# MicahZoltu/lodestar

Hardware: AMD Instinct MI355X
Metric: verified signature sets/sec (mainnet attestation mix) (higher is better)
Workload: dtype u32 (381-bit Montgomery; device products on 14x28-bit limbs); 1 GPU; c3: gossip attestation flood, 6 slot(s) per batch, 7 batches in flight per GPU; slots_per_batch=6, sets_per_gpu=116736, jobs_per_gpu=104448, pubkeys_per_gpu=1683456, parallelism=dp1 (sets sharded), exchange=False, inflight=7, world_size_seen=1, pubkeys=indices into the GPU-resident table, signing_roots_per_gpu=6918

## Files before the change

lodestar_amd/csrc/lb_engine.hip:

```cpp
#include <hip/hip_runtime.h>
#include <hip/hip_ext.h>
#include <stdio.h>
#include <stdlib.h>
#include <string.h>
#include <sys/random.h>

#include <algorithm>
#include <chrono>
#include <cstdio>
#include <cstdlib>
#include <atomic>
#include <mutex>
#include <string>
#include <vector>

#include "lb_kernels.h"
#include "lb_engine_impl.h"
#include "lb_kdecl.h"
#include "lb_search_plan.h"

#define LB_ABI_VERSION 1

namespace {
const char* const kStageNames[kStages] = {"decode_sigs", "dedup",   "hash_map", "hash_finish", "pk_chunks",
// ... 635 lines not shown
                         e->bacc.as<uint32_t>(), bcap, e->bsum.as<uint32_t>(), nb);
    hipLaunchKernelGGL(k_msm_window_g8, dim3(n_inst * W), dim3(256), 0, st, e->bsum.as<uint32_t>(), nb,
                       e->wsum.as<uint32_t>(), n_inst * W);
    if (W == LB_MSM_W)
      hipLaunchKernelGGL(k_msm_horner_g8<LB_MSM_W>, dim3((n_inst + 7) / 8), dim3(64), 0, st, e->wsum.as<uint32_t>(),
                         n_inst, out, n_out, out0);
    else
      hipLaunchKernelGGL(k_msm_horner_g8<LB_SMSM_W>, dim3((n_inst + 7) / 8), dim3(64), 0, st, e->wsum.as<uint32_t>(),
                         n_inst, out, n_out, out0);
    return hipGetLastError();
  }
  hipLaunchKernelGGL(k_msm_buckets, dim3(nblk(nb)), dim3(LB_TPB), 0, st, e->bch.as<uint32_t>(), e->bacc.as<uint32_t>(),
                     bcap, e->bsum.as<uint32_t>(), nb);
  if (W == LB_MSM_W)
    hipLaunchKernelGGL(k_msm_reduce<LB_MSM_W>, dim3(n_inst), dim3(64 * LB_MSM_W), 0, st, e->bsum.as<uint32_t>(), nb, out,
                       n_out, out0);
  else
    hipLaunchKernelGGL(k_msm_reduce<LB_SMSM_W>, dim3(n_inst), dim3(64 * LB_SMSM_W), 0, st, e->bsum.as<uint32_t>(), nb,
                       out, n_out, out0);
  return hipGetLastError();
}

static hipError_t per_root_chain(lb_engine* e, uint32_t n, uint32_t nuh, uint32_t mu) {
  hipStream_t s1 = e->stream;
  const uint32_t* nu = e->n_u.as<uint32_t>();
  const bool row = e->alone && e->row_fe;
  const bool row_roots = row && nuh <= e->row_max;
  {
    stage_scope sc(e, ST_GSUM, s1);
    const uint32_t nch = nuh + n / e->gchunk;
    if (e->alone)
      hipLaunchKernelGGL(k_gsum_wave, dim3(nblk(nch)), dim3(LB_TPB), 0, s1, n, nu, e->gch.as<uint32_t>(),
                         e->chunk_beg.as<uint32_t>(), e->chunk_end.as<uint32_t>(), e->chunk_root.as<uint32_t>(),
                         e->members.as<uint32_t>(), e->set_live.as<uint32_t>(), e->rpk.as<uint32_t>(), e->gacc.as<uint32_t>());
    else
      hipLaunchKernelGGL(k_gsum_chunks, dim3(nblk(nch)), dim3(LB_TPB), 0, s1, n, nu,
                         e->gch.as<uint32_t>(), e->chunk_beg.as<uint32_t>(), e->chunk_end.as<uint32_t>(),
                         e->members.as<uint32_t>(), e->set_live.as<uint32_t>(), e->rpk.as<uint32_t>(), e->gacc.as<uint32_t>());
    hipLaunchKernelGGL(k_gsum_final, dim3(nblk_inv(nuh)), dim3(LB_INV_TPB), 0, s1, n, nu, e->gch.as<uint32_t>(),
                       e->gacc.as<uint32_t>(), e->gp_aff.as<uint32_t>(), e->gp_inf.as<uint32_t>(),
                       e->alone ? 1u : 0u);
  }
  {
    stage_scope sc(e, ST_MILLER, s1);
    const bool shared = e->miller_form == 1 ||
                        (e->miller_form == 0 && !device_alone(e));
    if (row_roots) {
      hipLaunchKernelGGL(k_miller_row, dim3(nuh), dim3(LBR_NT), 0, s1, n, mu, nu, e->gp_aff.as<uint32_t>(),
                         e->gp_inf.as<uint32_t>(), e->h_aff.as<uint32_t>(), e->treeP.as<uint32_t>());
    } else if (nuh <= e->miller_wave_max) {
      hipLaunchKernelGGL(k_miller_wave, dim3(nuh), dim3(64), 0, s1, n, mu, nu, e->gp_aff.as<uint32_t>(),
                         e->gp_inf.as<uint32_t>(), e->h_aff.as<uint32_t>(), e->treeP.as<uint32_t>());
    } else if (shared) {
      hipError_t r = e->park.ensure((size_t)2 * 72 * 4 * n);
      if (r != hipSuccess) return r;
      if (nuh <= e->miller_lds3_max)
        hipLaunchKernelGGL(k_miller_lane<3>, dim3(nblk(nuh)), dim3(LB_TPB), 0, s1, n, mu, nu, e->gp_aff.as<uint32_t>(),
                           e->gp_inf.as<uint32_t>(), e->h_aff.as<uint32_t>(), e->treeP.as<uint32_t>(),
                           e->park.as<uint32_t>());
      else
        hipLaunchKernelGGL(k_miller_lane<2>, dim3(nblk(nuh)), dim3(LB_TPB), 0, s1, n, mu, nu, e->gp_aff.as<uint32_t>(),
                           e->gp_inf.as<uint32_t>(), e->h_aff.as<uint32_t>(), e->treeP.as<uint32_t>(),
                           e->park.as<uint32_t>());
    } else {
      hipLaunchKernelGGL(k_miller_g8, dim3((nuh + LBG_ROOTS - 1) / LBG_ROOTS), dim3(64 * LBG_WAVES), 0, s1, n, mu, nu,
                         e->gp_aff.as<uint32_t>(), e->gp_inf.as<uint32_t>(), e->h_aff.as<uint32_t>(),
                         e->treeP.as<uint32_t>());
    }
  }
  {
    stage_scope sc(e, ST_TREE_P, s1);
    for (uint32_t lo = mu / 2; lo >= 1; lo /= 2) {
      if (row && lo <= e->row_max)
        hipLaunchKernelGGL(k_tree_up_row, dim3(lo), dim3(LBR_NT), 0, s1, mu, lo, nu, e->treeP.as<uint32_t>());
      else
        hipLaunchKernelGGL(k_tree_up_U, dim3(lo), dim3(64), 0, s1, mu, lo, nu, e->treeP.as<uint32_t>());
    }
  }
  return hipGetLastError();
}

static int32_t run_pipeline(lb_engine* e, lb_batch* b, const uint64_t* scalars, uint32_t& mj, uint32_t& mu,
                            bool unblinded) {
  const uint32_t n = b->n_sets, nj = b->n_jobs;
  e->partial_serial = 0;
  e->alone = device_alone(e);
  e->gchunk = e->alone ? LB_GROUP_CHUNK_WAVE : LB_GROUP_CHUNK;
  const bool row = e->alone && e->row_fe;
  const bool row_small = row && n <= e->row_max;
  const bool one_unblinded = n == 1 && !scalars && unblinded;
  int st = fill_scalars(e, n, scalars, unblinded);
  if (st != LB_OK) return st;
  mj = 1;
  while (mj < nj) mj <<= 1;
  mu = 1;
  while (mu < n) mu <<= 1;
  const uint32_t mt = mj > mu ? mj : mu;
  const uint32_t ns = n ? n : 1;
  uint32_t cap = 64;
  while (cap < 2 * ns) cap <<= 1;
  LB_HIP(e->scalars.ensure((size_t)ns * 8));
  LB_HIP(e->sig_aff.ensure((size_t)ns * sizeof(g2a)));
  LB_HIP(e->sig_inf.ensure((size_t)ns * 4));
  LB_HIP(e->sig_status.ensure((size_t)ns * 4));
  LB_HIP(e->q.ensure((size_t)ns * 2 * sizeof(g2j)));
  LB_HIP(e->h_aff.ensure((size_t)ns * sizeof(g2a)));
  LB_HIP(e->rpk.ensure((size_t)ns * sizeof(g1j)));
// ... 872 lines not shown
```

lodestar_amd/csrc/lb_field.h:

```cpp
#pragma once
#include "lb_common.h"
#include "lb_consts.h"

struct fp {
  uint32_t v[12];
};
struct fp2 {
  fp c0, c1;
};
struct fp6 {
  fp2 c0, c1, c2;
};
struct fp12 {
  fp6 c0, c1;
};

LB_HD fp fp_load(const uint32_t* c) {
  fp r;
  LB_UNROLL for (int i = 0; i < 12; i++) r.v[i] = c[i];
  return r;
}
LB_HD fp2 fp2_load(const uint32_t* c) {
  fp2 r;
  r.c0 = fp_load(c);
// ... 451 lines not shown
  const uint32_t P28[14] = {LB_P28_0, LB_P28_1, LB_P28_2, LB_P28_3, LB_P28_4,  LB_P28_5,  LB_P28_6,
                            LB_P28_7, LB_P28_8, LB_P28_9, LB_P28_10, LB_P28_11, LB_P28_12, LB_P28_13};
  typedef unsigned __int128 u128;
  const u128 lim = (u128)~0ull;
  fp28_chk_in(a), fp28_chk_in(b);
  if (c) fp28_chk_in(*c), fp28_chk_in(*d);
  u128 col[29];
  for (int k = 0; k < 29; k++) col[k] = 0;
  for (int i = 0; i < 14; i++) {
    for (int j = 0; j < 14; j++) {
      col[i + j] += (u128)a.ub[i] * b.ub[j] + (u128)0x0fffffffu * P28[j];
      if (c) col[i + j] += (u128)c->ub[i] * d->ub[j];
    }
    LB_CHK_ASSERT(col[i] <= lim);
    col[i + 1] += col[i] >> 28;
  }
  for (int k = 14; k < 28; k++) {
    LB_CHK_ASSERT(col[k] <= lim);
    col[k + 1] += col[k] >> 28;
  }
  const double s = a.vb * b.vb + (c ? c->vb * d->vb : 0.0);
  const double vb = (1.0 + s / 2520.0) * (1.0 + 1e-9);
  LB_CHK_ASSERT(vb < 2520.0);
  fp28_chk_set(r, vb);
}
#endif

struct fp2_28 {
  fp28 c0, c1;
};
LB_HD fp28 fp28_add(const fp28& a, const fp28& b) {
  fp28 r;
  LB_UNROLL for (int k = 0; k < 14; k++) {
    r.l[k] = a.l[k] + b.l[k];
    LB_CHK(r.ub[k] = a.ub[k] + b.ub[k]; LB_CHK_ASSERT(r.ub[k] <= 0xffffffffull);)
  }
  LB_CHK(r.vb = a.vb + b.vb;)
  return r;
}
template <int N>
LB_HD fp28 fp28_muls(const fp28& a) {
  fp28 r;
  LB_UNROLL for (int k = 0; k < 14; k++) {
    r.l[k] = N == 3 ? (a.l[k] << 1) + a.l[k] : a.l[k] << (N == 2 ? 1 : N == 4 ? 2 : 3);
    LB_CHK(r.ub[k] = N * a.ub[k]; LB_CHK_ASSERT(r.ub[k] <= 0xffffffffull);)
  }
  LB_CHK(r.vb = N * a.vb;)
  return r;
}
template <uint32_t C, int S>
LB_HD fp28 fp28_kminus(const fp28& b) {
  constexpr uint32_t K[14] = LB_K28(C, S);
  fp28 r;
  LB_UNROLL for (int k = 0; k < 14; k++) {
    r.l[k] = K[k] - b.l[k];
    LB_CHK(LB_CHK_ASSERT(b.ub[k] <= K[k]); r.ub[k] = K[k];)
  }
  LB_CHK(r.vb = C;)
  return r;
}
template <uint32_t C, int S>
LB_HD fp28 fp28_sub(const fp28& a, const fp28& b) {
  constexpr uint32_t K[14] = LB_K28(C, S);
  fp28 r;
  LB_UNROLL for (int k = 0; k < 14; k++) {
    r.l[k] = a.l[k] + K[k] - b.l[k];
    LB_CHK(LB_CHK_ASSERT(b.ub[k] <= K[k]); r.ub[k] = a.ub[k] + K[k]; LB_CHK_ASSERT(r.ub[k] <= 0xffffffffull);)
  }
  LB_CHK(r.vb = a.vb + C;)
  return r;
}
LB_HD fp28 fp28_norm(const fp28& a) {
  fp28 r;
  uint32_t c = 0;
  LB_CHK(uint64_t cb = 0;)
  LB_UNROLL for (int k = 0; k < 13; k++) {
    const uint32_t t = a.l[k] + c;
    LB_CHK(LB_CHK_ASSERT(a.ub[k] + cb <= 0xffffffffull); cb = (a.ub[k] + cb) >> 28;)
    r.l[k] = t & 0x0fffffffu;
    c = t >> 28;
  }
  r.l[13] = a.l[13] + c;
  LB_CHK(const uint64_t top = a.ub[13] + cb; fp28_chk_set(r, a.vb); if (top < r.ub[13]) r.ub[13] = top;)
  return r;
}
LB_HD fp28 fp28_mulx(const fp28& a, const fp28& b) {
#if defined(__HIP_DEVICE_COMPILE__)
  __builtin_amdgcn_sched_barrier(0);
#endif
  fp28 r = fp28_mul_raw(a, b);
#if defined(__HIP_DEVICE_COMPILE__)
  __builtin_amdgcn_sched_barrier(0);
#endif
  LB_CHK(fp28_chk_mac(a, b, nullptr, nullptr, r);)
  return r;
}
LB_HD fp28 fp28_mac2(const fp28& a, const fp28& b, const fp28& c, const fp28& d) {
  const uint32_t P28[14] = {LB_P28_0, LB_P28_1, LB_P28_2, LB_P28_3, LB_P28_4,  LB_P28_5,  LB_P28_6,
                            LB_P28_7, LB_P28_8, LB_P28_9, LB_P28_10, LB_P28_11, LB_P28_12, LB_P28_13};
#if defined(__HIP_DEVICE_COMPILE__)
  __builtin_amdgcn_sched_barrier(0);
#endif
  uint64_t acc[28];
  LB_UNROLL for (int k = 0; k < 28; k++) acc[k] = 0;
  LB_UNROLL for (int i = 0; i < 14; i++) {
    LB_UNROLL for (int j = 0; j < 14; j++) {
      LB_COL_CHK(acc[i + j], a.l[i], b.l[j]);
      acc[i + j] += (uint64_t)a.l[i] * b.l[j];
    }
    LB_UNROLL for (int j = 0; j < 14; j++) {
      LB_COL_CHK(acc[i + j], c.l[i], d.l[j]);
      acc[i + j] += (uint64_t)c.l[i] * d.l[j];
    }
    const uint32_t m = ((uint32_t)acc[i] * LB_PINV28) & 0x0fffffffu;
    LB_UNROLL for (int j = 0; j < 14; j++) {
      LB_COL_CHK(acc[i + j], m, P28[j]);
      acc[i + j] += (uint64_t)m * P28[j];
// ... 59 lines not shown
  }
  return fp_reduce_once(o, 0u);
}
LB_HD bool fp28_is_zero(const fp28& a) {
  const uint32_t P28[14] = {LB_P28_0, LB_P28_1, LB_P28_2, LB_P28_3, LB_P28_4,  LB_P28_5,  LB_P28_6,
                            LB_P28_7, LB_P28_8, LB_P28_9, LB_P28_10, LB_P28_11, LB_P28_12, LB_P28_13};
  LB_CHK(fp28_chk_in(a); LB_CHK_ASSERT(a.vb < 2520.0);)
  uint64_t acc[28];
  LB_UNROLL for (int k = 0; k < 28; k++) acc[k] = k < 14 ? a.l[k] : 0;
  LB_UNROLL for (int i = 0; i < 14; i++) {
    const uint32_t m = ((uint32_t)acc[i] * LB_PINV28) & 0x0fffffffu;
    LB_UNROLL for (int j = 0; j < 14; j++) acc[i + j] += (uint64_t)m * P28[j];
    acc[i + 1] += acc[i] >> 28;
  }
  uint32_t z = 0, e = 0;
  LB_UNROLL for (int k = 0; k < 14; k++) {
    const uint32_t t = k < 13 ? ((uint32_t)acc[14 + k] & 0x0fffffffu) : (uint32_t)acc[27];
    if (k < 13) acc[15 + k] += acc[14 + k] >> 28;
    z |= t;
    e |= t ^ P28[k];
  }
  return z == 0 || e == 0;
}

LB_HD fp2_28 fp2_28_add(const fp2_28& a, const fp2_28& b) { return fp2_28{fp28_add(a.c0, b.c0), fp28_add(a.c1, b.c1)}; }
template <int N>
LB_HD fp2_28 fp2_28_muls(const fp2_28& a) {
  return fp2_28{fp28_muls<N>(a.c0), fp28_muls<N>(a.c1)};
}
template <uint32_t C, int S>
LB_HD fp2_28 fp2_28_sub(const fp2_28& a, const fp2_28& b) {
  return fp2_28{fp28_sub<C, S>(a.c0, b.c0), fp28_sub<C, S>(a.c1, b.c1)};
}
LB_HD fp2_28 fp2_28_norm(const fp2_28& a) { return fp2_28{fp28_norm(a.c0), fp28_norm(a.c1)}; }
template <uint32_t C, int S>
LB_HD fp2_28 fp2_28_mul(const fp2_28& a, const fp2_28& b) {
  const fp28 nb1 = fp28_kminus<C, S>(b.c1);
  fp2_28 r;
  r.c0 = fp28_mac2(a.c0, b.c0, a.c1, nb1);
  r.c1 = fp28_mac2(a.c0, b.c1, a.c1, b.c0);
  return r;
}
template <uint32_t C, int S>
LB_HD fp2_28 fp2_28_sqr(const fp2_28& a) {
  fp2_28 r;
  r.c0 = fp28_mulx(fp28_add(a.c0, a.c1), fp28_sub<C, S>(a.c0, a.c1));
  r.c1 = fp28_mulx(fp28_muls<2>(a.c0), a.c1);
  return r;
}
LB_HD bool fp2_28_is_zero(const fp2_28& a) { return fp28_is_zero(a.c0) & fp28_is_zero(a.c1); }
LB_HD fp2_28 fp2_28_from_fp2(const fp2& a) { return fp2_28{fp28_from_fp(a.c0), fp28_from_fp(a.c1)}; }
LB_HD fp2_28 fp2_28_from_fp2_shift(const fp2& a) { return fp2_28{fp28_from_fp_shift(a.c0), fp28_from_fp_shift(a.c1)}; }
LB_HD fp2 fp2_28_to_fp2(const fp2_28& a) { return fp2{fp28_to_fp(a.c0), fp28_to_fp(a.c1)}; }

template <bool kInlMul = false>
LB_HD fp fp_pow_const_i(fp a, const uint32_t* e, int top_bit) {
  if constexpr (kInlMul) return fp_pow_const_28(a, e, top_bit);
  fp tab[8];
  tab[0] = a;
  const fp a2 = fp_sqr(a);
  LB_UNROLL for (int k = 1; k < 8; k++) tab[k] = fp_mul(tab[k - 1], a2);
  auto bit = [&](int i) -> uint32_t { return (e[i >> 5] >> (i & 31)) & 1u; };
  fp r = fp_zero();
  bool first = true;
  int i = top_bit;
  while (i >= 0) {
    if (!bit(i)) {
      r = fp_sqr(r);
      i--;
      continue;
    }
    int j = i - 3 > 0 ? i - 3 : 0;
    while (!bit(j)) j++;
    uint32_t val = 0;
    for (int k = i; k >= j; k--) val = (val << 1) | bit(k);
    if (first) {
      r = lb_tab8(tab, val >> 1);
      first = false;
    } else {
      for (int k = i; k >= j; k--) r = fp_sqr(r);
      r = fp_mul(r, lb_tab8(tab, val >> 1));
    }
    i = j - 1;
  }
  return r;
}

LB_HD bool lb_is_one_plain(const uint32_t* x) {
  uint32_t t = x[0] ^ 1u;
  LB_UNROLL for (int i = 1; i < 12; i++) t |= x[i];
  return t == 0;
}
LB_HD int lb_ctz32(uint32_t x) {
#if defined(__HIP_DEVICE_COMPILE__)
  return __builtin_ctz(x);
#else
  return __builtin_ctz(x);
#endif
}
LB_HD void lb_shr(uint32_t* u, int k) {
  LB_UNROLL for (int j = 0; j < 11; j++) u[j] = (u[j] >> k) | (u[j + 1] << (32 - k));
  u[11] >>= k;
}
LB_HD bool lb_geq(const uint32_t* a, const uint32_t* b) {
  uint32_t br = 0;
  LB_UNROLL for (int j = 0; j < 12; j++) (void)LB_SUBC(a[j], b[j], br, &br);
// ... 585 lines not shown
```

lodestar_amd/csrc/lb_kernels.h:

```cpp
#pragma once
#include "lb_serial.h"
#include "lb_h2c.h"
#include "lb_pairing.h"

#define LB_TPB 64
#ifndef LB_MINW
#define LB_MINW 1
#endif
#ifndef LB_MINW_DEC
#define LB_MINW_DEC 2
#endif
#ifndef LB_MINW_SUB
#define LB_MINW_SUB LB_MINW_DEC
#endif
#ifndef LB_MINW_MSM
#define LB_MINW_MSM 1
#endif
#ifndef LB_MINW_GSUM
#define LB_MINW_GSUM 1
#endif
typedef fpi lb_g1f;
typedef fp2i lb_g2f;
typedef jac<lb_g2f> g2jm;
#ifndef LB_MINW_G1
// ... 972 lines not shown
    ok = g2_aff_in_subgroup_i(P);
  } else {
    const rfp2 Z2 = f_sqr(Z);
    const rfp2 sx = f_mul(fl_conj(px), fl_in(fp2_load(LB_PSI_CX), t2));
    const rfp2 sy = f_mul(fl_conj(py), fl_in(fp2_load(LB_PSI_CY), t2));
    ok = fp2_eq(fl_out(f_mul(sx, Z2)), fl_out(X)) && fp2_eq(fl_out(f_mul(f_mul(sy, Z2), Z)), fl_out(f_neg(Y)));
  }
  if (!ok && threadIdx.x == 0) sig_status[i] = LB_POINT_NOT_IN_GROUP;
}
#endif
#if LB_KG(13)
__global__ void __launch_bounds__(64) k_sig_blind_w4(uint32_t n, const uint32_t* __restrict__ sig_aff,
                                                    const uint64_t* __restrict__ scalars,
                                                    const uint32_t* __restrict__ sig_inf, uint32_t* __restrict__ terms) {
  const uint32_t i = blockIdx.x;
  if (i >= n) return;
  const uint64_t w = scalars[i];
  g2j r = jac_infinity<fp2>();
  if (!sig_inf[i] && w != 0) {
    const g2a S = soa_ld<g2a>(sig_aff, n, i);
    const rfp2* t2p = nullptr;
    const rfp* t1p = nullptr;
    const rfp2 x1 = fl_in(S.x, t2p), y1 = fl_in(S.y, t2p);
    const rfp c2x = fl_in(fp_load(LB_PSI2_CX), t1p), c2y = fl_in(fp_load(LB_PSI2_CY), t1p);
    const rfp c4x = fl_in(fp_load(LB_PSI4_CX), t1p), c4y = fl_in(fp_load(LB_PSI4_CY), t1p);
    const rfp2 x2 = fl_mulb(x1, c2x), y2 = f_neg(fl_mulb(y1, c2y));
    const rfp2 x3 = fl_mulb(x1, c4x), y3 = f_neg(fl_mulb(y1, c4y));
    const uint32_t k0 = (uint32_t)w, k1 = (uint32_t)(w >> 32);
    auto digit = [&](int b) { return ((k0 >> b) & 1u) | (((k1 >> b) & 1u) << 1); };
    int b = 31;
    while (b > 0 && digit(b) == 0) b--;
    const uint32_t d0 = digit(b);
    rfp2 X = d0 == 1u ? x1 : (d0 == 2u ? x2 : x3), Y = d0 == 1u ? y1 : (d0 == 2u ? y2 : y3), Z;
    f_set_one(Z);
#pragma clang loop unroll(disable)
    for (b--; b >= 0; b--) {
      w4_g2_dbl(X, Y, Z);
      const uint32_t d = digit(b);
      if (d != 0u) w4_g2_madd(X, Y, Z, d == 1u ? x1 : (d == 2u ? x2 : x3), d == 1u ? y1 : (d == 2u ? y2 : y3));
    }
    r = g2j{fl_out(X), fl_out(Y), fl_out(Z)};
  }
  if (threadIdx.x == 0) soa_st(terms, n, i, r);
}
#endif

typedef __attribute__((address_space(3))) uint32_t lds_w;
template <int NL>
struct lane_lds {
  lds_w* L;
  uint32_t* g;
  uint32_t n, u;
  int lane;
  __device__ __forceinline__ void put(int k, const fp6& v) const {
    const uint32_t* w = reinterpret_cast<const uint32_t*>(&v);
    if (k < NL)
      LB_UNROLL for (int i = 0; i < 72; i++) L[(k * 72 + i) * 64 + lane] = w[i];
    else
      LB_UNROLL for (int i = 0; i < 72; i++) g[((size_t)(k - 2) * 72 + i) * n + u] = w[i];
    __asm__ volatile("" ::: "memory");
  }
  __device__ __forceinline__ fp6 get(int k) const {
    __asm__ volatile("" ::: "memory");
    fp6 v;
    uint32_t* w = reinterpret_cast<uint32_t*>(&v);
    if (k < NL)
      LB_UNROLL for (int i = 0; i < 72; i++) w[i] = L[(k * 72 + i) * 64 + lane];
    else
      LB_UNROLL for (int i = 0; i < 72; i++) w[i] = g[((size_t)(k - 2) * 72 + i) * n + u];
    return v;
  }
};
template <class S_t>
__device__ __forceinline__ void lane_f_sqr(const S_t& S) {
  fp6 s1, s2;
  {
    const fp6 a0 = S.get(0), a1 = S.get(1);
    S.put(2, fp6_mul_inl(a0, a1));
    s1 = fp6_add(a0, a1);
    s2 = fp6_add(a0, fp6_mul_v(a1));
  }
  const fp6 c0 = fp6_mul_inl(s1, s2);
  const fp6 t = S.get(2);
  S.put(0, fp6_sub(fp6_sub(c0, t), fp6_mul_v(t)));
  S.put(1, fp6_add(t, t));
}
template <class S_t>
__device__ __forceinline__ void lane_f_line(const S_t& S, const fp2& l0, const fp2& l2, const fp2& l3) {
  fp6 s;
  {
    const fp6 a1 = S.get(1);
    S.put(2, fp6_mul_1(a1, l3));
    const fp6 a0 = S.get(0);
    s = fp6_add(a0, a1);
    S.put(0, fp6_mul_01(a0, l0, l2));
  }
  const fp6 c1 = fp6_mul_01(s, l0, fp2_add(l2, l3));
  const fp6 t0 = S.get(0), t1 = S.get(2);
  S.put(1, fp6_sub(fp6_sub(c1, t0), t1));
  S.put(0, fp6_add(t0, fp6_mul_v(t1)));
}
#if LB_KG(4)
template <int NL>
__global__ void __launch_bounds__(LB_TPB, 1) k_miller_lane(uint32_t n, uint32_t m,
                                                           const uint32_t* __restrict__ n_u,
                                                           const uint32_t* __restrict__ gp_aff,
                                                           const uint32_t* __restrict__ gp_inf,
                                                           const uint32_t* __restrict__ h_aff,
                                                           uint32_t* __restrict__ treeP, uint32_t* __restrict__ tpark) {
  static_assert(LB_TPB == 64, "one wave per block: 64 lanes of LDS slots");
  __shared__ uint32_t lds[NL * 72 * 64];
  const uint32_t u = lb_tid();
  if (u >= *n_u) return;
  const lane_lds<NL> S{(lds_w*)lds, tpark, n, u, (int)threadIdx.x};
  S.put(0, fp6_one());
  S.put(1, fp6_zero());
  if (!gp_inf[u]) {
    auto park_t = [&](const g2j& T) { S.put(3, *reinterpret_cast<const fp6*>(&T)); };
    auto unpark_t = [&]() {
      const fp6 v = S.get(3);
      return *reinterpret_cast<const g2j*>(&v);
    };
    {
      const g2a Q = soa_ld<g2a>(h_aff, n, u);
      park_t(g2j{Q.x, Q.y, fp2_one()});
    }
    bool first = true;
#pragma clang loop unroll(disable)
    for (int i = 62; i >= 0; i--) {
      if (!first) lane_f_sqr(S);
      first = false;
      fp2 l0, l2, l3;
      {
        g2j T = unpark_t();
        const g1a P = soa_ld<g1a>(gp_aff, n, u);
        miller_dbl(T, l0, l2, l3, P.x, P.y);
        park_t(T);
      }
      lane_f_line(S, l0, l2, l3);
      if ((LB_X_ABS >> i) & 1ull) {
        {
          g2j T = unpark_t();
          const g1a P = soa_ld<g1a>(gp_aff, n, u);
          miller_add(T, soa_ld<g2a>(h_aff, n, u), l0, l2, l3, P.x, P.y);
          park_t(T);
        }
        lane_f_line(S, l0, l2, l3);
      }
    }
    S.put(1, fp6_neg(S.get(1)));
  }
  LB_UNROLL for (int h = 0; h < 2; h++) {
    const fp6 v = S.get(h);
    const uint32_t* w = reinterpret_cast<const uint32_t*>(&v);
    LB_UNROLL for (int i = 0; i < 72; i++) treeP[(size_t)(72 * h + i) * (2 * m) + m + u] = w[i];
  }
}
#endif

#if LB_KG(5)
__global__ void __launch_bounds__(64) k_miller_wave(uint32_t n, uint32_t m, const uint32_t* __restrict__ n_u,
                                                    const uint32_t* __restrict__ gp_aff,
                                                    const uint32_t* __restrict__ gp_inf,
                                                    const uint32_t* __restrict__ h_aff, uint32_t* __restrict__ treeP) {
  LBW_SHARED_MILLER(S);
  const uint32_t u = blockIdx.x;
  if (u >= *n_u) return;
  const int lane = threadIdx.x;
  w_init_consts(S, LBW_MILLER_COUNT, LBW_MILLER_FIRST);
  const bool inf = gp_inf[u] != 0;
  if (inf) {
    w_set_one(S, LBW_A(0));
  } else {
    if (lane < 6) {
      const uint32_t* base = lane < 2 ? gp_aff + (size_t)12 * lane * n : h_aff + (size_t)12 * (lane - 2) * n;
      fp v;
      LB_UNROLL for (int w = 0; w < 12; w++) v.v[w] = base[(size_t)w * n + u];
      w_st(S, LBW_PT + lane, v);
    }
    w_sync();
    w_miller(S, LBW_A(0));
  }
  w_store_soa12(S, LBW_A(0), treeP, 2 * m, m + u);
}
#endif

#define LB_GROUP_CHUNK 32
#ifndef LB_GROUP_CHUNK_WAVE
#define LB_GROUP_CHUNK_WAVE 4
#endif
#ifndef LB_MSM_CHUNK
#define LB_MSM_CHUNK 16
#endif
__device__ __forceinline__ bool msg_eq(const uint8_t* __restrict__ msgs, uint32_t a, uint32_t b) {
  const uint4* x = reinterpret_cast<const uint4*>(msgs + (size_t)32 * a);
  const uint4* y = reinterpret_cast<const uint4*>(msgs + (size_t)32 * b);
  const uint4 x0 = x[0], x1 = x[1], y0 = y[0], y1 = y[1];
  return ((x0.x ^ y0.x) | (x0.y ^ y0.y) | (x0.z ^ y0.z) | (x0.w ^ y0.w) | (x1.x ^ y1.x) | (x1.y ^ y1.y) |
          (x1.z ^ y1.z) | (x1.w ^ y1.w)) == 0u;
}
__device__ __forceinline__ uint32_t msg_hash(const uint8_t* __restrict__ msgs, uint32_t i, uint64_t key) {
  const uint4* x = reinterpret_cast<const uint4*>(msgs + (size_t)32 * i);
  const uint4 a = x[0], b = x[1];
  const uint32_t w[8] = {a.x, a.y, a.z, a.w, b.x, b.y, b.z, b.w};
  uint64_t h = key;
  LB_UNROLL for (int k = 0; k < 8; k++) {
    h = (h ^ w[k]) * 0x9E3779B97F4A7C15ull;
    h ^= h >> 29;
// ... 1452 lines not shown
```

lodestar_amd/csrc/lb_pairing.h:

```cpp
#pragma once
#include "lb_curve.h"

template <bool kInl = false>
LB_HD void miller_dbl(g2j& T, fp2& l0, fp2& l2, fp2& l3, const fp& xP, const fp& yP) {
  fp2 X = T.x, Y = T.y, Z = T.z;
  fp2 A = lean2_mul<kInl>(X, Y);
  fp2 B = lean2_sqr<kInl>(Y);
  fp2 C = lean2_sqr<kInl>(Z);
  fp2 E = fp2_mul3(fp2_dbl(fp2_dbl(fp2_mul_xi(C))));
  fp2 F = fp2_mul3(E);
  fp2 H = fp2_sub(lean2_sqr<kInl>(fp2_add(Y, Z)), fp2_add(B, C));
  fp2 XX3 = fp2_mul3(lean2_sqr<kInl>(X));
  l0 = fp2_sub(B, E);
  l2 = fp2_neg(fp2{lean_mul<kInl>(XX3.c0, xP), lean_mul<kInl>(XX3.c1, xP)});
  l3 = fp2{lean_mul<kInl>(H.c0, yP), lean_mul<kInl>(H.c1, yP)};
  T.x = fp2_dbl(lean2_mul<kInl>(A, fp2_sub(B, F)));
  T.y = fp2_sub(lean2_sqr<kInl>(fp2_add(B, F)), fp2_mul3(fp2_dbl(fp2_dbl(lean2_sqr<kInl>(E)))));
  T.z = fp2_dbl(fp2_dbl(lean2_mul<kInl>(B, H)));
}

template <bool kInl = false>
LB_HD void miller_add(g2j& T, const g2a& Q, fp2& l0, fp2& l2, fp2& l3, const fp& xP, const fp& yP) {
  fp2 theta = fp2_sub(T.y, lean2_mul<kInl>(Q.y, T.z));
  fp2 lam = fp2_sub(T.x, lean2_mul<kInl>(Q.x, T.z));
// ... 9 lines not shown
  T.x = lean2_mul<kInl>(lam, H);
  T.y = fp2_sub(lean2_mul<kInl>(theta, fp2_sub(G, H)), lean2_mul<kInl>(E, T.y));
  T.z = lean2_mul<kInl>(T.z, E);
}

LB_NI fp12 miller_loop(g1a P, g2a Q) {
  g2j T;
  T.x = Q.x;
  T.y = Q.y;
  T.z = fp2_one();
  fp2 l0, l2, l3;
  fp12 f = fp12_one();
  bool first = true;
  for (int i = 62; i >= 0; i--) {
    if (!first) f = fp12_sqr(f);
    miller_dbl(T, l0, l2, l3, P.x, P.y);
    if (first) {
      f = fp12_one();
      first = false;
    }
    f = fp12_mul_line(f, l0, l2, l3);
    if ((LB_X_ABS >> i) & 1ull) {
      miller_add(T, Q, l0, l2, l3, P.x, P.y);
      f = fp12_mul_line(f, l0, l2, l3);
    }
  }
  return fp12_conj(f);
}

LB_HD fp12 miller_loop_inl(const g1a& P, const g2a& Q) {
  g2j T;
  T.x = Q.x;
  T.y = Q.y;
  T.z = fp2_one();
  fp2 l0, l2, l3;
  fp12 f = fp12_one();
  bool first = true;
  for (int i = 62; i >= 0; i--) {
    if (!first) f = fp12_sqr_inl(f);
    miller_dbl(T, l0, l2, l3, P.x, P.y);
    if (first) {
      f = fp12_one();
      first = false;
    }
    f = fp12_mul_line_inl(f, l0, l2, l3);
    if ((LB_X_ABS >> i) & 1ull) {
      miller_add(T, Q, l0, l2, l3, P.x, P.y);
      f = fp12_mul_line_inl(f, l0, l2, l3);
    }
  }
  return fp12_conj(f);
}

LB_NI fp12 fp12_pow_xabs(fp12 a) {
  fp12 r = a;
  for (int i = 62; i >= 0; i--) {
    r = fp12_sqr(r);
    if ((LB_X_ABS >> i) & 1ull) r = fp12_mul(r, a);
  }
  return r;
}

LB_NI fp12 final_exponentiation(fp12 f) {
  fp12 t = fp12_mul(fp12_conj(f), fp12_inv(f));
  t = fp12_mul(fp12_frob2(t), t);
  fp12 a = fp12_conj(fp12_mul(fp12_pow_xabs(t), t));
  a = fp12_conj(fp12_mul(fp12_pow_xabs(a), a));
  fp12 b = fp12_mul(fp12_conj(fp12_pow_xabs(a)), fp12_frob(a));
  fp12 c = fp12_pow_xabs(fp12_pow_xabs(b));
  c = fp12_mul(fp12_mul(c, fp12_frob2(b)), fp12_conj(b));
  fp12 t3 = fp12_mul(fp12_sqr(t), t);
  return fp12_mul(c, t3);
}
```

Measured before the change: 12.42 million sets/s.

## Port lane Miller loop to lazy-reduced 28-bit limb arithmetic in LDS slots

Rewrites the shared-LDS Miller loop kernel to keep the accumulator and the G2 point in the 14x28-bit limb representation, with lazily reduced fp2/fp6 arithmetic whose per-operation bound constants are tracked explicitly. LDS and parking slots are reorganised into 28-word fp2 coefficients (84 words per fp6), and the loop is restructured into f_sqr28/f_line28 working slot-by-slot. The aim is to avoid repeated conversions to full Montgomery form and to cut reduction work per field operation. The cost is a larger LDS and park footprint per lane, and correctness now depends on hand-chosen bound constants.

```diff
diff --git a/lodestar_amd/csrc/lb_engine.hip b/lodestar_amd/csrc/lb_engine.hip
--- a/lodestar_amd/csrc/lb_engine.hip
+++ b/lodestar_amd/csrc/lb_engine.hip
@@ -711,7 +711,7 @@
       hipLaunchKernelGGL(k_miller_wave, dim3(nuh), dim3(64), 0, s1, n, mu, nu, e->gp_aff.as<uint32_t>(),
                          e->gp_inf.as<uint32_t>(), e->h_aff.as<uint32_t>(), e->treeP.as<uint32_t>());
     } else if (shared) {
-      hipError_t r = e->park.ensure((size_t)2 * 72 * 4 * n);
+      hipError_t r = e->park.ensure((size_t)2 * 84 * 4 * n);
       if (r != hipSuccess) return r;
       if (nuh <= e->miller_lds3_max)
         hipLaunchKernelGGL(k_miller_lane<3>, dim3(nblk(nuh)), dim3(LB_TPB), 0, s1, n, mu, nu, e->gp_aff.as<uint32_t>(),
diff --git a/lodestar_amd/csrc/lb_field.h b/lodestar_amd/csrc/lb_field.h
--- a/lodestar_amd/csrc/lb_field.h
+++ b/lodestar_amd/csrc/lb_field.h
@@ -527,6 +527,7 @@
 LB_HD fp28 fp28_kminus(const fp28& b) {
   constexpr uint32_t K[14] = LB_K28(C, S);
   fp28 r;
+  LB_CHK(if (b.ub[13] > K[13]) fprintf(stderr, "K = %u p does not cover a value of %.2f p\n", C, b.vb);)
   LB_UNROLL for (int k = 0; k < 14; k++) {
     r.l[k] = K[k] - b.l[k];
     LB_CHK(LB_CHK_ASSERT(b.ub[k] <= K[k]); r.ub[k] = K[k];)
@@ -538,6 +539,7 @@
 LB_HD fp28 fp28_sub(const fp28& a, const fp28& b) {
   constexpr uint32_t K[14] = LB_K28(C, S);
   fp28 r;
+  LB_CHK(if (b.ub[13] > K[13]) fprintf(stderr, "K = %u p does not cover a value of %.2f p\n", C, b.vb);)
   LB_UNROLL for (int k = 0; k < 14; k++) {
     r.l[k] = a.l[k] + K[k] - b.l[k];
     LB_CHK(LB_CHK_ASSERT(b.ub[k] <= K[k]); r.ub[k] = a.ub[k] + K[k]; LB_CHK_ASSERT(r.ub[k] <= 0xffffffffull);)
@@ -703,6 +705,85 @@
 LB_HD fp2_28 fp2_28_from_fp2(const fp2& a) { return fp2_28{fp28_from_fp(a.c0), fp28_from_fp(a.c1)}; }
 LB_HD fp2_28 fp2_28_from_fp2_shift(const fp2& a) { return fp2_28{fp28_from_fp_shift(a.c0), fp28_from_fp_shift(a.c1)}; }
 LB_HD fp2 fp2_28_to_fp2(const fp2_28& a) { return fp2{fp28_to_fp(a.c0), fp28_to_fp(a.c1)}; }
+
+struct fp6_28 {
+  fp2_28 c0, c1, c2;
+};
+template <uint32_t C, int S>
+LB_HD fp2_28 fp2_28_mul_xi(const fp2_28& a) {
+  return fp2_28{fp28_sub<C, S>(a.c0, a.c1), fp28_add(a.c0, a.c1)};
+}
+template <uint32_t C, int S>
+LB_HD fp2_28 fp2_28_kminus(const fp2_28& a) {
+  return fp2_28{fp28_kminus<C, S>(a.c0), fp28_kminus<C, S>(a.c1)};
+}
+LB_HD fp6_28 fp6_28_add(const fp6_28& a, const fp6_28& b) {
+  return fp6_28{fp2_28_add(a.c0, b.c0), fp2_28_add(a.c1, b.c1), fp2_28_add(a.c2, b.c2)};
+}
+template <uint32_t C, int S>
+LB_HD fp6_28 fp6_28_sub(const fp6_28& a, const fp6_28& b) {
+  return fp6_28{fp2_28_sub<C, S>(a.c0, b.c0), fp2_28_sub<C, S>(a.c1, b.c1), fp2_28_sub<C, S>(a.c2, b.c2)};
+}
+template <uint32_t C, int S>
+LB_HD fp6_28 fp6_28_mul_v(const fp6_28& a) {
+  return fp6_28{fp2_28_mul_xi<C, S>(a.c2), a.c0, a.c1};
+}
+LB_HD fp6_28 fp6_28_norm(const fp6_28& a) { return fp6_28{fp2_28_norm(a.c0), fp2_28_norm(a.c1), fp2_28_norm(a.c2)}; }
+template <uint32_t CB, uint32_t CB2, uint32_t CT, uint32_t CX, uint32_t CXT, class A, class B, class O>
+LB_HD void fp6_28_mul_to(A&& a, B&& b, O&& out) {
+  const fp2_28 t0 = fp2_28_mul<CB, 28>(a(0), b(0));
+  const fp2_28 t1 = fp2_28_mul<CB, 28>(a(1), b(1));
+  const fp2_28 t2 = fp2_28_mul<CB, 28>(a(2), b(2));
+  {
+    const fp2_28 m = fp2_28_mul<CB2, 29>(fp2_28_add(a(1), a(2)), fp2_28_add(b(1), b(2)));
+    const fp2_28 x = fp2_28_sub<CT, 29>(m, fp2_28_add(t1, t2));
+    out(0, fp2_28_norm(fp2_28_add(fp2_28_mul_xi<CX, 31>(x), t0)));
+  }
+  {
+    const fp2_28 m = fp2_28_mul<CB2, 29>(fp2_28_add(a(0), a(1)), fp2_28_add(b(0), b(1)));
+    out(1, fp2_28_norm(fp2_28_add(fp2_28_sub<CT, 29>(m, fp2_28_add(t0, t1)), fp2_28_mul_xi<CXT, 28>(t2))));
+  }
+  {
+    const fp2_28 m = fp2_28_mul<CB2, 29>(fp2_28_add(a(0), a(2)), fp2_28_add(b(0), b(2)));
+    out(2, fp2_28_norm(fp2_28_add(fp2_28_sub<CT, 29>(m, fp2_28_add(t0, t2)), t1)));
+  }
+}
+template <uint32_t CB0, uint32_t CB1, uint32_t CBS, uint32_t CT, uint32_t CX, class A, class O>
+LB_HD void fp6_28_mul_01_to(A&& a, const fp2_28& b0, const fp2_28& b1, const fp2_28& bs, O&& out) {
+  const fp2_28 t0 = fp2_28_mul<CB0, 28>(a(0), b0);
+  const fp2_28 t1 = fp2_28_mul<CB1, 28>(a(1), b1);
+  out(1, fp2_28_norm(fp2_28_sub<CT, 29>(fp2_28_mul<CBS, 28>(fp2_28_add(a(0), a(1)), bs), fp2_28_add(t0, t1))));
+  out(0, fp2_28_norm(fp2_28_add(fp2_28_mul_xi<CX, 28>(fp2_28_mul<CB1, 28>(a(2), b1)), t0)));
+  out(2, fp2_28_add(fp2_28_mul<CB0, 28>(a(2), b0), t1));
+}
+template <uint32_t CB1, uint32_t CX, class A, class O>
+LB_HD void fp6_28_mul_1_to(A&& a, const fp2_28& b1, O&& out) {
+  out(0, fp2_28_norm(fp2_28_mul_xi<CX, 28>(fp2_28_mul<CB1, 28>(a(2), b1))));
+  out(1, fp2_28_mul<CB1, 28>(a(0), b1));
+  out(2, fp2_28_mul<CB1, 28>(a(1), b1));
+}
+LB_HD const fp2_28& fp6_28_at(const fp6_28& a, int i) { return i == 0 ? a.c0 : i == 1 ? a.c1 : a.c2; }
+LB_HD fp2_28& fp6_28_at(fp6_28& a, int i) { return i == 0 ? a.c0 : i == 1 ? a.c1 : a.c2; }
+template <uint32_t CB, uint32_t CB2, uint32_t CT, uint32_t CX, uint32_t CXT>
+LB_HD fp6_28 fp6_28_mul(const fp6_28& a, const fp6_28& b) {
+  fp6_28 r;
+  fp6_28_mul_to<CB, CB2, CT, CX, CXT>([&](int i) { return fp6_28_at(a, i); }, [&](int i) { return fp6_28_at(b, i); },
+                                      [&](int i, const fp2_28& v) { fp6_28_at(r, i) = v; });
+  return r;
+}
+template <uint32_t CB0, uint32_t CB1, uint32_t CBS, uint32_t CT, uint32_t CX>
+LB_HD fp6_28 fp6_28_mul_01(const fp6_28& a, const fp2_28& b0, const fp2_28& b1) {
+  fp6_28 r;
+  fp6_28_mul_01_to<CB0, CB1, CBS, CT, CX>([&](int i) { return fp6_28_at(a, i); }, b0, b1, fp2_28_norm(fp2_28_add(b0, b1)),
+                                          [&](int i, const fp2_28& v) { fp6_28_at(r, i) = v; });
+  return r;
+}
+template <uint32_t CB1, uint32_t CX>
+LB_HD fp6_28 fp6_28_mul_1(const fp6_28& a, const fp2_28& b1) {
+  fp6_28 r;
+  fp6_28_mul_1_to<CB1, CX>([&](int i) { return fp6_28_at(a, i); }, b1, [&](int i, const fp2_28& v) { fp6_28_at(r, i) = v; });
+  return r;
+}
 
 template <bool kInlMul = false>
 LB_HD fp fp_pow_const_i(fp a, const uint32_t* e, int top_bit) {
diff --git a/lodestar_amd/csrc/lb_kernels.h b/lodestar_amd/csrc/lb_kernels.h
--- a/lodestar_amd/csrc/lb_kernels.h
+++ b/lodestar_amd/csrc/lb_kernels.h
@@ -1048,54 +1048,25 @@
   uint32_t* g;
   uint32_t n, u;
   int lane;
-  __device__ __forceinline__ void put(int k, const fp6& v) const {
+  __device__ __forceinline__ void put2(int k, int i, const fp2_28& v) const {
     const uint32_t* w = reinterpret_cast<const uint32_t*>(&v);
     if (k < NL)
-      LB_UNROLL for (int i = 0; i < 72; i++) L[(k * 72 + i) * 64 + lane] = w[i];
+      LB_UNROLL for (int j = 0; j < 28; j++) L[(k * 84 + i * 28 + j) * 64 + lane] = w[j];
     else
-      LB_UNROLL for (int i = 0; i < 72; i++) g[((size_t)(k - 2) * 72 + i) * n + u] = w[i];
+      LB_UNROLL for (int j = 0; j < 28; j++) g[((size_t)(k - 2) * 84 + i * 28 + j) * n + u] = w[j];
     __asm__ volatile("" ::: "memory");
   }
-  __device__ __forceinline__ fp6 get(int k) const {
+  __device__ __forceinline__ fp2_28 get2(int k, int i) const {
     __asm__ volatile("" ::: "memory");
-    fp6 v;
+    fp2_28 v;
     uint32_t* w = reinterpret_cast<uint32_t*>(&v);
     if (k < NL)
-      LB_UNROLL for (int i = 0; i < 72; i++) w[i] = L[(k * 72 + i) * 64 + lane];
+      LB_UNROLL for (int j = 0; j < 28; j++) w[j] = L[(k * 84 + i * 28 + j) * 64 + lane];
     else
-      LB_UNROLL for (int i = 0; i < 72; i++) w[i] = g[((size_t)(k - 2) * 72 + i) * n + u];
+      LB_UNROLL for (int j = 0; j < 28; j++) w[j] = g[((size_t)(k - 2) * 84 + i * 28 + j) * n + u];
     return v;
   }
 };
-template <class S_t>
-__device__ __forceinline__ void lane_f_sqr(const S_t& S) {
-  fp6 s1, s2;
-  {
-    const fp6 a0 = S.get(0), a1 = S.get(1);
-    S.put(2, fp6_mul_inl(a0, a1));
-    s1 = fp6_add(a0, a1);
-    s2 = fp6_add(a0, fp6_mul_v(a1));
-  }
-  const fp6 c0 = fp6_mul_inl(s1, s2);
-  const fp6 t = S.get(2);
-  S.put(0, fp6_sub(fp6_sub(c0, t), fp6_mul_v(t)));
-  S.put(1, fp6_add(t, t));
-}
-template <class S_t>
-__device__ __forceinline__ void lane_f_line(const S_t& S, const fp2& l0, const fp2& l2, const fp2& l3) {
-  fp6 s;
-  {
-    const fp6 a1 = S.get(1);
-    S.put(2, fp6_mul_1(a1, l3));
-    const fp6 a0 = S.get(0);
-    s = fp6_add(a0, a1);
-    S.put(0, fp6_mul_01(a0, l0, l2));
-  }
-  const fp6 c1 = fp6_mul_01(s, l0, fp2_add(l2, l3));
-  const fp6 t0 = S.get(0), t1 = S.get(2);
-  S.put(1, fp6_sub(fp6_sub(c1, t0), t1));
-  S.put(0, fp6_add(t0, fp6_mul_v(t1)));
-}
 #if LB_KG(4)
 template <int NL>
 __global__ void __launch_bounds__(LB_TPB, 1) k_miller_lane(uint32_t n, uint32_t m,
@@ -1105,51 +1076,22 @@
                                                            const uint32_t* __restrict__ h_aff,
                                                            uint32_t* __restrict__ treeP, uint32_t* __restrict__ tpark) {
   static_assert(LB_TPB == 64, "one wave per block: 64 lanes of LDS slots");
-  __shared__ uint32_t lds[NL * 72 * 64];
+  static_assert(sizeof(fp2_28) == 28 * sizeof(uint32_t), "a slot coefficient is 28 words");
+  __shared__ uint32_t lds[NL * 84 * 64];
   const uint32_t u = lb_tid();
   if (u >= *n_u) return;
   const lane_lds<NL> S{(lds_w*)lds, tpark, n, u, (int)threadIdx.x};
-  S.put(0, fp6_one());
-  S.put(1, fp6_zero());
+  S.put2(0, 0, fp2_28{fp28_one(), fp28_zero()});
+  LB_UNROLL for (int c = 1; c < 6; c++) S.put2(c / 3, c % 3, fp2_28{fp28_zero(), fp28_zero()});
   if (!gp_inf[u]) {
-    auto park_t = [&](const g2j& T) { S.put(3, *reinterpret_cast<const fp6*>(&T)); };
-    auto unpark_t = [&]() {
-      const fp6 v = S.get(3);
-      return *reinterpret_cast<const g2j*>(&v);
-    };
-    {
-      const g2a Q = soa_ld<g2a>(h_aff, n, u);
-      park_t(g2j{Q.x, Q.y, fp2_one()});
-    }
-    bool first = true;
+    miller_lane28(S, [&]() { return soa_ld<g1a>(gp_aff, n, u); }, [&]() { return soa_ld<g2a>(h_aff, n, u); });
+    LB_UNROLL for (int i = 0; i < 3; i++) S.put2(1, i, fp2_28_kminus<LB_M28_CONJ_C, 28>(S.get2(1, i)));
+  }
 #pragma clang loop unroll(disable)
-    for (int i = 62; i >= 0; i--) {
-      if (!first) lane_f_sqr(S);
-      first = false;
-      fp2 l0, l2, l3;
-      {
-        g2j T = unpark_t();
-        const g1a P = soa_ld<g1a>(gp_aff, n, u);
-        miller_dbl(T, l0, l2, l3, P.x, P.y);
-        park_t(T);
-      }
-      lane_f_line(S, l0, l2, l3);
-      if ((LB_X_ABS >> i) & 1ull) {
-        {
-          g2j T = unpark_t();
-          const g1a P = soa_ld<g1a>(gp_aff, n, u);
-          miller_add(T, soa_ld<g2a>(h_aff, n, u), l0, l2, l3, P.x, P.y);
-          park_t(T);
-        }
-        lane_f_line(S, l0, l2, l3);
-      }
-    }
-    S.put(1, fp6_neg(S.get(1)));
-  }
-  LB_UNROLL for (int h = 0; h < 2; h++) {
-    const fp6 v = S.get(h);
+  for (int c = 0; c < 6; c++) {
+    const fp2 v = fp2_28_to_fp2(S.get2(c / 3, c % 3));
     const uint32_t* w = reinterpret_cast<const uint32_t*>(&v);
-    LB_UNROLL for (int i = 0; i < 72; i++) treeP[(size_t)(72 * h + i) * (2 * m) + m + u] = w[i];
+    LB_UNROLL for (int i = 0; i < 24; i++) treeP[(size_t)(24 * c + i) * (2 * m) + m + u] = w[i];
   }
 }
 #endif
diff --git a/lodestar_amd/csrc/lb_pairing.h b/lodestar_amd/csrc/lb_pairing.h
--- a/lodestar_amd/csrc/lb_pairing.h
+++ b/lodestar_amd/csrc/lb_pairing.h
@@ -85,6 +85,156 @@
   return fp12_conj(f);
 }
 
+#define LB_M28_VF00 10.0
+#define LB_M28_VF01 14.0
+#define LB_M28_VF02 6.0
+#define LB_M28_VF10 20.0
+#define LB_M28_VF11 27.0
+#define LB_M28_VF12 17.0
+#define LB_M28_VX 8.0
+#define LB_M28_VY 72.0
+#define LB_M28_VZ 8.0
+#define LB_M28_CONJ_C 28
+#if defined(LB_FP28_CHECK)
+static inline void fp2_28_chk_assume(fp2_28& a, double vb) { fp28_chk_assume(a.c0, vb), fp28_chk_assume(a.c1, vb); }
+template <class S_t>
+static inline void miller28_chk_assume(const S_t& S) {
+  const double vf[2][3] = {{LB_M28_VF00, LB_M28_VF01, LB_M28_VF02}, {LB_M28_VF10, LB_M28_VF11, LB_M28_VF12}};
+  const double vt[3] = {LB_M28_VX, LB_M28_VY, LB_M28_VZ};
+  for (int k = 0; k < 2; k++)
+    for (int i = 0; i < 3; i++) {
+      fp2_28 v = S.get2(k, i);
+      fp2_28_chk_assume(v, vf[k][i]);
+      S.put2(k, i, v);
+    }
+  for (int i = 0; i < 3; i++) {
+    fp2_28 v = S.get2(3, i);
+    fp2_28_chk_assume(v, vt[i]);
+    S.put2(3, i, v);
+  }
+}
+#endif
+
+LB_HD void miller_dbl28(fp2_28& X, fp2_28& Y, fp2_28& Z, fp2_28& l0, fp2_28& l2, fp2_28& l3, const fp28& xP,
+                        const fp28& yP) {
+  const fp2_28 A = fp2_28_mul<73, 28>(X, Y);
+  const fp2_28 B = fp2_28_sqr<73, 28>(Y);
+  const fp2_28 C = fp2_28_sqr<9, 28>(Z);
+  const fp2_28 E = fp2_28_norm(fp2_28_muls<3>(fp2_28_norm(fp2_28_muls<4>(fp2_28_mul_xi<2, 28>(C)))));
+  const fp2_28 H = fp2_28_sub<11, 29>(fp2_28_sqr<81, 28>(fp2_28_norm(fp2_28_add(Y, Z))), fp2_28_add(B, C));
+  const fp2_28 XX3 = fp2_28_muls<3>(fp2_28_sqr<9, 28>(X));
+  l0 = fp2_28_norm(fp2_28_sub<38, 28>(B, E));
+  l2 = fp2_28_norm(fp2_28_kminus<2, 28>(fp2_28{fp28_mulx(XX3.c0, xP), fp28_mulx(XX3.c1, xP)}));
+  l3 = fp2_28{fp28_mulx(H.c0, yP), fp28_mulx(H.c1, yP)};
+  const fp2_28 F = fp2_28_muls<3>(E);
+  X = fp2_28_norm(fp2_28_muls<2>(fp2_28_mul<123, 31>(A, fp2_28_sub<113, 30>(B, F))));
+  Y = fp2_28_norm(fp2_28_sub<39, 30>(fp2_28_sqr<122, 28>(fp2_28_norm(fp2_28_add(B, F))),
+                                     fp2_28_muls<3>(fp2_28_norm(fp2_28_muls<4>(fp2_28_sqr<38, 28>(E))))));
+  Z = fp2_28_norm(fp2_28_muls<4>(fp2_28_mul<10, 28>(H, B)));
+}
+
+LB_HD void miller_add28(fp2_28& X, fp2_28& Y, fp2_28& Z, const fp2_28& Qx, const fp2_28& Qy, fp2_28& l0, fp2_28& l2,
+                        fp2_28& l3, const fp28& xP, const fp28& yP) {
+  const fp2_28 theta = fp2_28_norm(fp2_28_sub<3, 28>(Y, fp2_28_mul<9, 28>(Qy, Z)));
+  const fp2_28 lam = fp2_28_norm(fp2_28_sub<3, 28>(X, fp2_28_mul<9, 28>(Qx, Z)));
+  l0 = fp2_28_norm(fp2_28_sub<4, 28>(fp2_28_mul<76, 28>(Qx, theta), fp2_28_mul<12, 28>(Qy, lam)));
+  l2 = fp2_28_norm(fp2_28_kminus<9, 28>(fp2_28{fp28_mulx(theta.c0, xP), fp28_mulx(theta.c1, xP)}));
+  l3 = fp2_28{fp28_mulx(lam.c0, yP), fp28_mulx(lam.c1, yP)};
+  const fp2_28 C = fp2_28_sqr<76, 28>(theta);
+  const fp2_28 D = fp2_28_sqr<12, 28>(lam);
+  const fp2_28 E = fp2_28_mul<2, 28>(lam, D);
+  const fp2_28 F = fp2_28_mul<10, 28>(Z, C);
+  const fp2_28 G = fp2_28_mul<2, 28>(X, D);
+  const fp2_28 H = fp2_28_norm(fp2_28_sub<3, 29>(fp2_28_add(E, F), fp2_28_muls<2>(G)));
+  X = fp2_28_mul<6, 28>(lam, H);
+  Y = fp2_28_norm(fp2_28_sub<2, 28>(fp2_28_mul<76, 28>(fp2_28_sub<6, 28>(G, H), theta), fp2_28_mul<2, 28>(Y, E)));
+  Z = fp2_28_mul<2, 28>(Z, E);
+}
+
+template <class S_t>
+LB_HD void f_sqr28(const S_t& S) {
+  auto at = [&](int k) { return [&S, k](int i) { return S.get2(k, i); }; };
+  fp6_28_mul_to<28, 48, 3, 5, 2>(at(0), at(1), [&](int i, const fp2_28& v) { S.put2(2, i, v); });
+  {
+    const fp2_28 b0 = S.get2(1, 0), b1 = S.get2(1, 1), b2 = S.get2(1, 2);
+    fp2_28 a = S.get2(0, 0);
+    S.put2(0, 0, fp2_28_norm(fp2_28_add(a, b0)));
+    S.put2(1, 0, fp2_28_norm(fp2_28_add(a, fp2_28_mul_xi<18, 28>(b2))));
+    a = S.get2(0, 1);
+    S.put2(0, 1, fp2_28_norm(fp2_28_add(a, b1)));
+    S.put2(1, 1, fp2_28_norm(fp2_28_add(a, b0)));
+    a = S.get2(0, 2);
+    S.put2(0, 2, fp2_28_norm(fp2_28_add(a, b2)));
+    S.put2(1, 2, fp2_28_norm(fp2_28_add(a, b1)));
+  }
+  fp6_28 c;
+  fp6_28_mul_to<46, 80, 5, 10, 3>(at(0), at(1), [&](int i, const fp2_28& v) { fp6_28_at(c, i) = v; });
+  {
+    const fp2_28 t0 = S.get2(2, 0), t1 = S.get2(2, 1), t2 = S.get2(2, 2);
+    S.put2(0, 0, fp2_28_norm(fp2_28_sub<26, 31>(c.c0, fp2_28_add(t0, fp2_28_mul_xi<8, 28>(t2)))));
+    S.put2(0, 1, fp2_28_norm(fp2_28_sub<22, 29>(c.c1, fp2_28_add(t1, t0))));
+    S.put2(0, 2, fp2_28_norm(fp2_28_sub<16, 29>(c.c2, fp2_28_add(t2, t1))));
+    S.put2(1, 0, fp2_28_norm(fp2_28_muls<2>(t0)));
+    S.put2(1, 1, fp2_28_norm(fp2_28_muls<2>(t1)));
+    S.put2(1, 2, fp2_28_norm(fp2_28_muls<2>(t2)));
+  }
+}
+template <class S_t>
+LB_HD void f_line28(const S_t& S, const fp2_28& l0, const fp2_28& l2, const fp2_28& l3) {
+  auto at = [&](int k) { return [&S, k](int i) { return S.get2(k, i); }; };
+  fp6_28_mul_1_to<4, 2>(at(1), l3, [&](int i, const fp2_28& v) { S.put2(2, i, v); });
+  LB_UNROLL for (int i = 0; i < 3; i++) S.put2(1, i, fp2_28_add(S.get2(0, i), S.get2(1, i)));
+  fp6_28_mul_01_to<48, 10, 57, 5, 2>(at(0), l0, l2, fp2_28_norm(fp2_28_add(l0, l2)),
+                                    [&](int i, const fp2_28& v) { S.put2(0, i, v); });
+  fp6_28 c;
+  {
+    const fp2_28 l23 = fp2_28_norm(fp2_28_add(l2, l3));
+    fp6_28_mul_01_to<48, 13, 61, 7, 2>(at(1), l0, l23, fp2_28_norm(fp2_28_add(l0, l23)),
+                                       [&](int i, const fp2_28& v) { fp6_28_at(c, i) = v; });
+  }
+  LB_UNROLL for (int i = 0; i < 3; i++) {
+    const fp2_28 t0 = S.get2(0, i);
+    S.put2(1, i, fp2_28_norm(fp2_28_sub<12, 30>(fp6_28_at(c, i), fp2_28_add(t0, S.get2(2, i)))));
+    S.put2(0, i, fp2_28_norm(fp2_28_add(t0, i == 0 ? fp2_28_mul_xi<2, 28>(S.get2(2, 2)) : S.get2(2, i - 1))));
+  }
+}
+
+template <class S_t, class LdP, class LdQ>
+LB_HD void miller_lane28(const S_t& S, LdP&& ldP, LdQ&& ldQ) {
+  {
+    const g2a Q = ldQ();
+    S.put2(3, 0, fp2_28_from_fp2(Q.x));
+    S.put2(3, 1, fp2_28_from_fp2(Q.y));
+    S.put2(3, 2, fp2_28{fp28_one(), fp28_zero()});
+  }
+  bool first = true;
+#pragma clang loop unroll(disable)
+  for (int i = 62; i >= 0; i--) {
+    LB_CHK(miller28_chk_assume(S);)
+    if (!first) f_sqr28(S);
+    first = false;
+    const int np = 1 + (int)((LB_X_ABS >> i) & 1ull);
+#pragma clang loop unroll(disable)
+    for (int pass = 0; pass < np; pass++) {
+      LB_CHK(if (pass) miller28_chk_assume(S);)
+      fp2_28 l0, l2, l3;
+      {
+        fp2_28 X = S.get2(3, 0), Y = S.get2(3, 1), Z = S.get2(3, 2);
+        const g1a P = ldP();
+        const fp28 xP = fp28_from_fp_shift(P.x), yP = fp28_from_fp_shift(P.y);
+        if (pass == 0) {
+          miller_dbl28(X, Y, Z, l0, l2, l3, xP, yP);
+        } else {
+          const g2a Q = ldQ();
+          miller_add28(X, Y, Z, fp2_28_from_fp2_shift(Q.x), fp2_28_from_fp2_shift(Q.y), l0, l2, l3, xP, yP);
+        }
+        S.put2(3, 0, X), S.put2(3, 1, Y), S.put2(3, 2, Z);
+      }
+      f_line28(S, l0, l2, l3);
+    }
+  }
+}
+
 LB_NI fp12 fp12_pow_xabs(fp12 a) {
   fp12 r = a;
   for (int i = 62; i >= 0; i--) {
```

New measurement: 13.09 million sets/s, median of 6. 5.4% higher.
